# fluent/chunkio

Hardware: AMD Instinct MI355X
Metric: device-resident CRC32 GB/s over N×400KB chunks; % HBM-read roofline (higher is better)
Workload: dtype u8

## Files before the change

chunkio_amd/csrc/cio_diag.h:

```cpp
#ifndef CIO_DIAG_H
#define CIO_DIAG_H



#ifndef CIO_DIAG_HALF_REPLICAS
#define CIO_DIAG_HALF_REPLICAS 0
#endif

#ifndef CIO_ABLATE_LOADS
#define CIO_ABLATE_LOADS 0
#endif

#ifndef CIO_DIAG_NO_ARRIVAL
#define CIO_DIAG_NO_ARRIVAL 0
#endif

#ifndef CIO_DIAG_TAIL
#define CIO_DIAG_TAIL 0
#endif

#ifndef CIO_LDS_FOLD
#define CIO_LDS_FOLD 1
#endif

#ifndef CIO_AHEAD_PEEL
#define CIO_AHEAD_PEEL 1
#endif

#ifndef CIO_SMALL_SLOTS
#define CIO_SMALL_SLOTS 1
#endif
#ifndef CIO_SMALL_EXP
#define CIO_SMALL_EXP 0
#endif

#ifndef CIO_HEAD_ALIGN
#define CIO_HEAD_ALIGN 128
#endif

#ifndef CIO_SMALL_NIBFOLD
#define CIO_SMALL_NIBFOLD 0
#endif


#ifndef CIO_SHA1_GROUP
#define CIO_SHA1_GROUP 4
#endif
#ifndef CIO_SHA1_SCHED_WAVES
#define CIO_SHA1_SCHED_WAVES 1
#endif
#ifndef CIO_SHA1_CHAINS
#define CIO_SHA1_CHAINS 32
#endif
#ifndef CIO_SHA1_READ_AT
#define CIO_SHA1_READ_AT 0
#endif
#ifndef CIO_SHA1_GROUP8
#define CIO_SHA1_GROUP8 8
#endif
// ... 26 lines not shown
```

chunkio_amd/csrc/cio_gpu_internal.h:

```cpp
#ifndef CIOA_GPU_INTERNAL_H
#define CIOA_GPU_INTERNAL_H

#include <hip/hip_runtime.h>
#include <stdint.h>
#include <string>
#include <vector>

#include "cio_diag.h"
#include "crc32_host.h"
#include "chunkio_amd/cio_crc32_gpu.h"

namespace cioa {

constexpr int kWave = 64;
constexpr int kGran = 16;
constexpr int kSub = 4;
constexpr int kRow = kWave * kGran;
constexpr int kStep = kSub * kRow;
constexpr int kThreads = 1024;
constexpr uint32_t kWavesPerWg = kThreads / kWave;
constexpr uint32_t kWfFold = 1u, kWfPublish = 2u;
constexpr int kX8Count = 2 * kStep;
constexpr uint32_t kSliceBytes = 131072;
constexpr uint32_t kShiftBytes = 32768;
// ... 5 lines not shown
    uint64_t a;
    uint64_t vlen;
    uint64_t g;
    uint32_t nsteps;
    uint32_t h;
    uint32_t npieces;
    uint32_t w0, w1;
    uint32_t pad;
};
static_assert(sizeof(ChunkDesc) == 48, "desc layout");

struct WaveStart {
    ChunkDesc d;
    uint32_t c;
    uint32_t pad[3];
};
static_assert(sizeof(WaveStart) == 64, "wave start layout");

struct DeviceState {
    bool ready = false;
    int cus = 0;
    uint32_t *slice = nullptr;
    uint32_t *shift = nullptr;
    uint32_t *x8 = nullptr;
    uint32_t *xinv8 = nullptr;
};

struct PlanHost {
    std::vector<ChunkDesc> desc;
    std::vector<WaveStart> ws;
    std::vector<uint32_t> tiny;
    std::vector<uint32_t> pfac;
    uint64_t S = 0, bytes = 0;
};

constexpr int kMaxDev = 64;

extern thread_local std::string g_err;
int fail(const char *what, hipError_t e = hipSuccess);
int device_state(DeviceState **out);
void plan_init(cio_crc32_plan *p, DeviceState *st, size_t n);
const char *plan_build(PlanHost &ph, const uint64_t *offs, const uint64_t *lens, size_t n, uint32_t W);
int plan_exec_impl(const cio_crc32_plan *p, const void *dev_base, const uint32_t *dev_seeds,
                   uint32_t *dev_out, const uint32_t *cid, hipStream_t s,
                   hipEvent_t ev0 = nullptr, hipEvent_t ev1 = nullptr);


constexpr int kDevHdrS = 0, kDevHdrNtiny = 1, kDevHdrBytes = 2, kDevHdrStatus = 3, kDevHdrWords = 4;
constexpr uint32_t kPlanBlock = 1024;

struct PlanBlockSum {
    uint64_t steps, bytes;
    uint32_t ntiny, err;
};

int devplan_launch_planner(const cio_crc32_devplan *dp, uint64_t dev_bytes, const uint64_t *dev_offs,
                           const uint64_t *dev_lens, size_t n, uint32_t *dev_status, hipStream_t s);
int devplan_crc_launch(const cio_crc32_plan *p, const unsigned long long *hdr, const void *dev_base,
                       const uint32_t *dev_seeds, uint32_t *dev_out, size_t n, hipStream_t s);

}

#define HIP_TRY(expr, what)                             \
    do {                                                   \
        hipError_t e_ = (expr);                            \
        if (e_ != hipSuccess) return cioa::fail(what, e_); \
    } while (0)

struct cio_crc32_plan {
    uint32_t n = 0;
    uint64_t S = 0;
    uint32_t W = 0;
    uint32_t grid = 0;
    uint32_t ntiny = 0;
    int prio = 1;
    uint64_t ustride = 0, ua0 = 0, uvlen = 0;
    uint32_t unsteps = 0, uh = 0;
    bool small = false;
    bool ahead = false;
    bool l64 = false;
    bool l64_small = false;
    unsigned long long *stamps = nullptr;
    uint64_t bytes = 0;
    cioa::ChunkDesc *desc = nullptr;
    cioa::WaveStart *wstart = nullptr;
    uint32_t *tiny = nullptr;
    unsigned long long *partials = nullptr;
    uint32_t *counters = nullptr;
    uint32_t *pfac = nullptr;
    cioa::DeviceState *st = nullptr;
};

struct cio_crc32_devplan {
    cio_crc32_plan *p = nullptr;
    uint32_t max_chunks = 0;
    cioa::PlanBlockSum *bsum = nullptr;
    unsigned long long *hdr = nullptr;
    uint64_t *roffs = nullptr, *rlens = nullptr;
    uint32_t *rcrc = nullptr;
};

#endif
```

chunkio_amd/csrc/crc32_gpu.hip:

```cpp

#include <hip/hip_runtime.h>
#include <stdint.h>
#include <string.h>
#include <stdio.h>
#include <stdlib.h>
#include <memory>
#include <mutex>
#include <shared_mutex>
#include <vector>
#include <string>
#include <algorithm>

#include <type_traits>

#include "cio_gpu_internal.h"

using namespace cioa;

namespace {


constexpr uint32_t cx_multmodp(uint32_t a, uint32_t b)
{
    uint32_t p = 0;
// ... 23 lines not shown
{
    uint32_t p = 0;
#pragma unroll
    for (int i = 31; i >= 0; --i) {
        p ^= b & (0u - ((a >> i) & 1u));
        b = (b >> 1) ^ (CIOA_POLY & (0u - (b & 1u)));
    }
    return p;
}

template <uint32_t C>
struct MulCols {
    uint32_t v[32];
    constexpr MulCols() : v{}
    {
        for (int j = 0; j < 32; ++j) {
            v[j] = cx_multmodp(C, 1u << j);
        }
    }
};

template <uint32_t C>
__device__ __forceinline__ uint32_t mulconst(uint32_t b)
{
    constexpr MulCols<C> K;
    uint32_t p[4] = {0u, 0u, 0u, 0u};
#pragma unroll
    for (int j = 0; j < 32; ++j) {
        p[j & 3] = __builtin_amdgcn_bitop3_b32(p[j & 3], 0u - ((b >> j) & 1u), K.v[j], 0x78);
    }
    return __builtin_amdgcn_bitop3_b32(p[0], p[1], p[2], 0x96) ^ p[3];
}

template <bool TREE>
__device__ __forceinline__ uint32_t fold_full(const uint32_t (&s)[kSub])
{
    constexpr uint32_t kXRow = cx_xpow8n(kRow);
    uint32_t h = s[0];
#pragma unroll
    for (int q = 1; q < kSub; ++q) {
        h = (TREE ? mulconst<kXRow>(h) : multmodp(kXRow, h)) ^ s[q];
    }
    return h;
}

__device__ __forceinline__ uint64_t div_u52(uint64_t x, uint64_t d)
{
    uint64_t q = (uint64_t) ((double) x / (double) d);
    if (q * d > x) {
        q -= 1;
    } else if ((q + 1) * d <= x) {
        q += 1;
    }
    return q;
}

__device__ __forceinline__ uint64_t uniform_u64(uint64_t v)
{
    const uint32_t lo = __builtin_amdgcn_readfirstlane((uint32_t) v);
    const uint32_t hi = __builtin_amdgcn_readfirstlane((uint32_t) (v >> 32));
    return ((uint64_t) hi << 32) | lo;
}

__device__ __forceinline__ uint64_t split_point(uint64_t w, uint64_t X, uint64_t W)
{
    if ((W & (W - 1)) == 0) {
// ... 113 lines not shown
}

constexpr int kE = 1024 / kThreads;
static_assert(kE == 1, "one slice and one shift entry per thread");

template <bool STAMPS = false, bool SHIFT = true>
__device__ __forceinline__ void write_tables(char *lds, uint32_t tid, const uint32_t (&tab_v)[kE],
                                             const uint32_t (&tab_sv)[kE], unsigned long long *ts = nullptr)
{
    const uint32_t k = tid >> 8, b = tid & 255u, lane = tid & 63u;
    const uint32_t srow = (k >> 1) * 65536u + b * 256u + (k & 1u) * 128u;
    const uint4 sv = make_uint4(tab_v[0], tab_v[0], tab_v[0], tab_v[0]);
#pragma unroll
    for (int i = 0; i < 8; ++i) {
        *reinterpret_cast<uint4 *>(lds + srow + 16u * ((lane + (uint32_t) i) & 7u)) = sv;
    }
    if (SHIFT) {
        const uint32_t hrow = kShiftOff + k * 8192u + b * 32u;
        const uint4 hv = make_uint4(tab_sv[0], tab_sv[0], tab_sv[0], tab_sv[0]);
#pragma unroll
        for (int i = 0; i < 2; ++i) {
            *reinterpret_cast<uint4 *>(lds + hrow + 16u * ((lane + (uint32_t) i) & 1u)) = hv;
        }
    }
    if (STAMPS) {
        ts[0] = __builtin_amdgcn_s_memrealtime();
        ts[1] = ts[0];
    }
}

struct StepRegs {
    uint4 q[kSub];
};

__device__ __forceinline__ void load_step(StepRegs &r, const uint8_t *cbase, uint64_t jj,
                                          uint64_t vlen, uint32_t lane)
{
    const uint64_t b0 = jj * kStep + (uint64_t) lane * kGran;
    const uint64_t last = (vlen - 1) & ~15ull;
#pragma unroll
    for (int q = 0; q < kSub; ++q) {
#if CIO_ABLATE_LOADS
        const uint64_t a = min(b0 + (uint64_t) q * kRow, last) + (uint64_t) (uintptr_t) cbase;
        r.q[q] = make_uint4((uint32_t) a, (uint32_t) (a >> 7) * 0x9E3779B9u, (uint32_t) a ^ 0x5bd1e995u,
                            (uint32_t) (a >> 3) + 0x7f4a7c15u);
#else
        r.q[q] = ldg16(cbase + min(b0 + (uint64_t) q * kRow, last));
#endif
    }
}

__device__ __forceinline__ void load_step64(StepRegs &r, const uint8_t *cbase, uint64_t jj, uint32_t lane)
{
    const uint64_t b0 = jj * kStep + (uint64_t) (64u * (lane & 15u) + 16u * (lane >> 4));
#pragma unroll
    for (int q = 0; q < kSub; ++q) {
        r.q[q] = ldg16(cbase + b0 + (uint64_t) q * kRow);
    }
}

__device__ __forceinline__ void load_step64c(StepRegs &r, const uint8_t *cbase, uint64_t jj, uint64_t vlen,
                                             uint32_t lane)
{
    const uint64_t b0 = jj * kStep + (uint64_t) (64u * (lane & 15u) + 16u * (lane >> 4));
    const uint64_t last = (vlen - 1) & ~15ull;
#pragma unroll
// ... 179 lines not shown
    }
}

__device__ __forceinline__ void tiny_chunks(const char *lds, uint32_t lb_lo, const uint8_t *base,
                                            const ChunkDesc *desc, const uint32_t *tiny,
                                            const uint32_t *seeds, uint32_t *out, const uint32_t *cid,
                                            uint32_t ntiny, uint32_t wave, uint32_t lane, uint32_t W)
{
    for (uint64_t t = (uint64_t) wave * kWave + lane; t < ntiny; t += (uint64_t) W * kWave) {
        const uint32_t c = tiny[t];
        const ChunkDesc d = desc[c];
        const uint32_t oc = cid ? cid[c] : c;
        uint32_t st = seeds ? seeds[oc] : 0xffffffffu;
        const uint8_t *p = base + d.a + d.h;
        const uint32_t len = (uint32_t) (d.vlen - d.h);
        for (uint32_t i = 0; i < len; ++i) {
            st = byte_step(lds, lb_lo, st, p[i]);
        }
        out[oc] = st;
    }
}

__device__ __forceinline__ void rotate_prio(uint32_t slot_group, uint64_t it)
{
    switch ((slot_group + (uint32_t) it) & 3u) {
    case 0: __builtin_amdgcn_s_setprio(0); break;
    case 1: __builtin_amdgcn_s_setprio(1); break;
    case 2: __builtin_amdgcn_s_setprio(2); break;
    default: __builtin_amdgcn_s_setprio(3); break;
    }
}

template <bool STAMPS = false, int PRIO = 1, bool UNIFORM = false, bool AHEAD = false, bool L64 = false,
          bool DEVHDR = false>
__global__ void __launch_bounds__(kThreads, 1)
crc32_stream_kernel(const uint8_t *base, uint64_t S_arg, uint64_t ustride, uint64_t ua0, uint64_t uvlen,
                    uint32_t W, uint32_t unsteps, uint32_t uh, uint32_t n,
                    const ChunkDesc *__restrict__ desc,
                    const WaveStart *__restrict__ wstart, const uint32_t *__restrict__ tiny,
                    const uint32_t *__restrict__ seeds, uint32_t *out, const uint32_t *__restrict__ cid,
                    unsigned long long *__restrict__ partials, uint32_t *__restrict__ counters,
                    const uint32_t *__restrict__ g_slice, const uint32_t *__restrict__ g_shift,
                    const uint32_t *__restrict__ g_x8, const uint32_t *__restrict__ pfac,
                    uint32_t ntiny_arg, unsigned long long *stamps)
{
    static_assert(!DEVHDR || (!STAMPS && !UNIFORM && !AHEAD), "device-planned batches take the general path");
    __shared__ __attribute__((aligned(16))) char lds[kLdsBytes];
    const uint32_t tid = threadIdx.x;
    const uint64_t S = DEVHDR ? uniform_u64(stamps[kDevHdrS]) : S_arg;
    const uint32_t ntiny = DEVHDR ? __builtin_amdgcn_readfirstlane((uint32_t) stamps[kDevHdrNtiny]) : ntiny_arg;
    unsigned long long t_entry = 0, t_tables = 0, t_stream = 0, t_first = 0, t_mid = 0, t_issued = 0;
    unsigned long long t_wt[2] = {0, 0}, t_step1 = 0, t_arrived = 0, t_bar1 = 0, t_bar2 = 0, t_folded = 0;
    if (STAMPS) {
        t_entry = __builtin_amdgcn_s_memrealtime();
    }

    const uint32_t wave = __builtin_amdgcn_readfirstlane(blockIdx.x * (kThreads / kWave) + (tid >> 6));
    const uint32_t lane = tid & 63u;
    const uint32_t lb_lo = (lane & kSliceRepMask) << 2;
    const uint32_t lb_hi = lb_lo | 0x10000u;
    const uint32_t lrep = (lane & kShiftRepMask) << 2;
    const uint32_t slot_group = __builtin_amdgcn_readfirstlane((tid >> 6) >> 2);
    const uint64_t g0 = uniform_u64(wave_start(wave, S, W));
    const uint64_t gend = uniform_u64(wave_start((uint64_t) wave + 1, S, W));
    const bool active = g0 < gend;

    uint32_t c = 0, lc = 0, c0 = 0;
    ChunkDesc d = {}, ld = {};
    uint32_t j = 0, lj = 0;
    uint64_t nload = 0;
    if (active) {
        if (UNIFORM) {
            c = __builtin_amdgcn_readfirstlane((uint32_t) split_point(wave, n, W));
            d.a = ua0 + (uint64_t) c * ustride;
            d.vlen = uvlen;
            d.g = (uint64_t) c * unsteps;
            d.nsteps = unsteps;
            d.h = uh;
        } else {
// ... 37 lines not shown
        if (nload > 0) {
            --nload;
            if (++lj == ld.nsteps && nload > 0) {
                if (UNIFORM) {
                    ++lc;
                    ld.a += ustride;
                    ld.g += unsteps;
                } else {
                    do {
                        ++lc;
                        ld = desc[lc];
                    } while (ld.nsteps == 0);
                }
                lj = 0;
            }
        }
    };

    auto build_tables = [&]() {
        uint32_t tab_v[kE], tab_sv[kE];
#pragma unroll
        for (int e = 0; e < kE; ++e) {
            const uint32_t idx = tid + (uint32_t) kThreads * e;
            table_entries<L64 ? cx_xpow8n(kStep - 64) : kXStepShift>(__builtin_amdgcn_readfirstlane(idx >> 8),
                                                                     idx & 255u, tab_v[e], tab_sv[e]);
        }
        write_tables<STAMPS>(lds, tid, tab_v, tab_sv, t_wt);
    };
    StepRegs cur, nxt;
    issue(cur);
    __builtin_amdgcn_sched_barrier(0);
    uint64_t ar_g = 0;
    uint32_t ar_ns = 0, ar_np = 0, ar_w0 = 0, ar_w1 = 0;
    if (CIO_DIAG_NO_ARRIVAL < 2) {
        const ChunkDesc &ad = desc[min(c0 + lane, n - 1)];
        ar_g = ad.g;
        ar_ns = ad.nsteps;
        ar_np = ad.npieces;
        ar_w0 = ad.w0;
        ar_w1 = ad.w1;
    }
    const uint32_t xl = g_x8[L64 ? 64u * (63u - lane) : kRow - (lane + 1) * kGran];
    const uint32_t *wwords = pfac + (W + n + 1);
    const uint32_t wfl = CIO_LDS_FOLD ? load_lane_u32(wwords + wave) : 0u;
    const uint32_t wlast = load_lane_u32(wwords + W + wave);
    uint32_t fold_own = 0, pub = 0;
    __builtin_amdgcn_sched_barrier(0);
    if (STAMPS) {
        t_issued = __builtin_amdgcn_s_memrealtime();
    }

    build_tables();
    __syncthreads();
    if (STAMPS) {
        t_tables = __builtin_amdgcn_s_memrealtime();
    }

    if (active) {
        uint32_t s[kSub] = {0u, 0u, 0u, 0u};
        uint64_t e[kSub] = {0ull, 0ull, 0ull, 0ull};
        uint32_t xlast = 0;
        uint32_t full_end = (uint32_t) (d.vlen / kStep);
        uint32_t seed = (j == 0) ? (seeds ? seeds[cid ? cid[c] : c] : 0xffffffffu) : 0u;
        uint64_t g = g0;

        auto crc_step = [&](StepRegs &r) -> bool {
            {
                if (L64 && (AHEAD || j < full_end)) {
                    const uint32_t h0 = step_shift(lds, lrep, s[0]);
                    transpose64(r);
                    if (j == 0) {
                        if (AHEAD) {
                            r.q[0].x ^= lane == 0 ? seed : 0u;
                        } else {
                            r.q[0] = head_fix(r.q[0], 4u * lane, d.h, seed);
                            r.q[1] = head_fix(r.q[1], 4u * lane + 1u, d.h, seed);
                            if (CIO_HEAD_ALIGN > 16) {
                                r.q[2] = head_fix(r.q[2], 4u * lane + 2u, d.h, seed);
                                r.q[3] = head_fix(r.q[3], 4u * lane + 3u, d.h, seed);
                            }
                        }
                    }
                    uint32_t st = block16(lds, lb_lo, lb_hi, h0, r.q[0]);
#pragma unroll
                    for (int q = 1; q < kSub; ++q) {
                        st = block16(lds, lb_lo, lb_hi, st, r.q[q]);
                    }
                    s[0] = st;
                    if (!AHEAD) {
                        e[0] = (uint64_t) j * kStep + 64ull * (lane + 1);
                    }
                } else if (L64) {
                    transpose64(r);
                    slow_compute64(lds, lb_lo, lb_hi, lrep, r, j, d.vlen, d.h, seed, lane, s[0], e[0]);
                } else if (AHEAD || j < full_end) {
                    uint32_t h[kSub];
#pragma unroll
                    for (int q = 0; q < kSub; ++q) {
                        h[q] = step_shift(lds, lrep, s[q]);
                    }
                    if (j == 0) {
                        r.q[0] = head_fix(r.q[0], lane, d.h, seed);
                    }
#pragma unroll
                    for (int q = 0; q < kSub; ++q) {
                        s[q] = block16(lds, lb_lo, lb_hi, h[q], r.q[q]);
                    }
                    if (!AHEAD) {
                        const uint64_t e0 = (uint64_t) j * kStep + (uint64_t) (lane + 1) * kGran;
#pragma unroll
                        for (int q = 0; q < kSub; ++q) {
                            e[q] = e0 + (uint64_t) q * kRow;
                        }
                    }
                } else {
                    slow_compute(lds, lb_lo, lb_hi, lrep, r, j, d.vlen, d.h, seed, lane, s, e);
                }
                ++g;
                ++j;
                return j == d.nsteps || g == gend;
            }
        };
        auto piece_end = [&]() {
            {
                {
                    uint32_t contrib;
                    if (AHEAD || j <= full_end) {
                        uint32_t a = j < d.nsteps ? xlast : xl;
                        asm volatile("" : "+v"(a));
                        contrib = multmodp(a, L64 ? s[0] : fold_full<UNIFORM>(s));
                    } else {
                        const uint64_t pend = min((uint64_t) j * kStep, d.vlen);
                        contrib = 0;
#pragma unroll
                        for (int q = 0; q < kSub; ++q) {
                            const uint64_t dist = e[q] < pend ? pend - e[q] : 0;
                            contrib ^= s[q] ? multmodp(g_x8[min(dist, (uint64_t) (kX8Count - 1))], s[q]) : 0u;
                        }
                    }
                    contrib = wave_xor(contrib);
                    if (d.g >= g0 && j == d.nsteps) {
                        if (lane == 0) {
                            out[cid ? cid[c] : c] = contrib;
                        }
                    } else if (j == d.nsteps && (wfl & kWfFold)) {
                        fold_own = contrib;
                    } else if (j < d.nsteps && (wfl & kWfPublish)) {
                        pub = contrib;
                    } else {
                        __hip_atomic_store(&partials[(uint64_t) wave + c], (unsigned long long) contrib,
                                           __ATOMIC_RELAXED, __HIP_MEMORY_SCOPE_AGENT);
                    }
                    if (g < gend) {
                        if (UNIFORM) {
                            ++c;
                            d.a += ustride;
                            d.g += unsteps;
                        } else {
                            do {
                                ++c;
                                d = desc[c];
                            } while (d.nsteps == 0);
                        }
                        j = 0;
#pragma unroll
                        for (int q = 0; q < kSub; ++q) {
                            s[q] = 0u;
                            e[q] = 0ull;
                        }
                        full_end = (uint32_t) (d.vlen / kStep);
                        seed = seeds ? seeds[cid ? cid[c] : c] : 0xffffffffu;
                    }
                }
            }
        };

        if (STAMPS) {
            t_first = __builtin_amdgcn_s_memrealtime();
        }
        const uint64_t iters = gend - g0;
        const uint64_t it_f = iters > 1 ? 1 : 0;
        if (AHEAD) {
            auto landed = [](StepRegs &r) {
                asm volatile("" : "+v"(r.q[0].x), "+v"(r.q[0].y), "+v"(r.q[0].z), "+v"(r.q[0].w),
                                  "+v"(r.q[1].x), "+v"(r.q[1].y), "+v"(r.q[1].z), "+v"(r.q[1].w),
                                  "+v"(r.q[2].x), "+v"(r.q[2].y), "+v"(r.q[2].z), "+v"(r.q[2].w),
                                  "+v"(r.q[3].x), "+v"(r.q[3].y), "+v"(r.q[3].z), "+v"(r.q[3].w));
            };
            auto half = [&](uint64_t it, StepRegs &use, StepRegs &fill, auto refill) {
                if (PRIO) {
                    rotate_prio(slot_group, it);
                }
                if (it == it_f) {
                    uint32_t wl = wlast;
                    asm volatile("" : "+v"(wl));
                    xlast = multmodp(wl, xl);
                }
                landed(use);
                if (decltype(refill)::value) {
                    issue(fill);
                }
                if (crc_step(use)) {
                    piece_end();
                }
                if (STAMPS && it == 0) {
                    t_step1 = __builtin_amdgcn_s_memrealtime();
                }
                if (STAMPS && it == iters / 2) {
                    t_mid = __builtin_amdgcn_s_memrealtime();
                }
            };
            using Refill = std::true_type;
#if CIO_AHEAD_PEEL
            using NoRefill = std::false_type;
            uint64_t it = 0;
            for (; it + 2 < iters; it += 2) {
                half(it, cur, nxt, Refill());
                half(it + 1, nxt, cur, Refill());
            }
            if (iters - it == 2) {
                half(it, cur, nxt, Refill());
                half(it + 1, nxt, cur, NoRefill());
            } else if (iters - it == 1) {
                half(it, cur, nxt, NoRefill());
            }
#else
            for (uint64_t it = 0; it < iters; it += 2) {
                half(it, cur, nxt, Refill());
                if (it + 1 < iters) {
                    half(it + 1, nxt, cur, Refill());
                }
            }
#endif
        }
        for (uint64_t it = 0; !AHEAD && it < iters; ++it) {
            if (PRIO) {
                rotate_prio(slot_group, it);
            }
            if (it == it_f) {
                uint32_t wl = wlast;
                asm volatile("" : "+v"(wl));
                xlast = multmodp(wl, xl);
            }
            const bool pe = crc_step(cur);
            if (STAMPS && it == 0) {
                t_step1 = __builtin_amdgcn_s_memrealtime();
            }
            if (nload > 0) {
                issue(cur);
            }
            if (pe) {
                piece_end();
            }
            if (STAMPS && it == iters / 2) {
                t_mid = __builtin_amdgcn_s_memrealtime();
            }
        }
        if (PRIO) {
            __builtin_amdgcn_s_setprio(0);
        }

        asm volatile("s_waitcnt vmcnt(0)" ::: "memory");
        if (STAMPS) {
            t_stream = __builtin_amdgcn_s_memrealtime();
        }
        for (uint32_t ac = c0; !CIO_DIAG_NO_ARRIVAL;) {
            const uint32_t idx = ac + lane;
            const bool inb = idx < n;
            const bool whole = ar_g >= g0 && ar_g + ar_ns <= gend;
            const bool local = CIO_LDS_FOLD && (ar_w0 ^ ar_w1) < kWavesPerWg;
            const bool member = inb && ar_ns != 0 && ar_g < gend && !whole && !local;
            const bool stop = !inb || (ar_ns != 0 && ar_g >= gend);
            uint32_t old = 0;
            if (member) {
                old = __hip_atomic_fetch_add(&counters[idx], 1u, __ATOMIC_RELAXED, __HIP_MEMORY_SCOPE_AGENT);
            }
            for (uint64_t fin = __ballot(member && old + 1 == ar_np); fin; fin &= fin - 1) {
                const uint32_t b = (uint32_t) __builtin_ctzll(fin);
                const uint32_t fc = ac + b;
                fold_chunk(__builtin_amdgcn_readlane(ar_w0, b), __builtin_amdgcn_readlane(ar_w1, b), fc,
                           cid ? cid[fc] : fc, lane, partials, pfac, out, counters);
            }
            if (__ballot(stop)) {
                break;
            }
            ac += kWave;
            const ChunkDesc &ad = desc[min(ac + lane, n - 1)];
            ar_g = ad.g;
            ar_ns = ad.nsteps;
            ar_np = ad.npieces;
            ar_w0 = ad.w0;
            ar_w1 = ad.w1;
        }
    }

    if (STAMPS) {
        t_arrived = __builtin_amdgcn_s_memrealtime();
    }
    tiny_chunks(lds, lb_lo, base, desc, tiny, seeds, out, cid, ntiny, wave, lane, W);
    if (CIO_LDS_FOLD) {
        __syncthreads();
        if (STAMPS) {
            t_bar1 = __builtin_amdgcn_s_memrealtime();
        }
        uint32_t *slot = reinterpret_cast<uint32_t *>(lds);
        if (lane == 0) {
            slot[tid >> 6] = pub;
        }
        __syncthreads();
        if (STAMPS) {
            t_bar2 = __builtin_amdgcn_s_memrealtime();
        }
        if (wfl & kWfFold) {
            const uint32_t nb = (wfl >> 8) & 0xffu;
            uint32_t a = 0;
            if (lane < kWavesPerWg && lane >= kWavesPerWg - nb) {
                a = slot[(tid >> 6) + lane - kWavesPerWg];
            }
            a = wave_xor(a) ^ fold_own;
            if (lane == 0) {
                out[cid ? cid[c0] : c0] = a;
            }
        }
        if (STAMPS) {
            t_folded = __builtin_amdgcn_s_memrealtime();
        }
    }
#if CIO_DIAG_TAIL == 1
    {
        const unsigned long long t0 = __builtin_amdgcn_s_memrealtime();
        while (__builtin_amdgcn_s_memrealtime() - t0 < 500) {
            __builtin_amdgcn_s_sleep(10);
        }
    }
#elif CIO_DIAG_TAIL == 2
    __syncthreads();
#endif
    if (STAMPS && lane == 0) {
        uint32_t hw_id, xcc_id;
        asm volatile("s_getreg_b32 %0, hwreg(HW_REG_HW_ID)" : "=s"(hw_id));
        asm volatile("s_getreg_b32 %0, hwreg(HW_REG_XCC_ID)" : "=s"(xcc_id));
        stamps[kStampWords * wave + 0] = t_entry;
        stamps[kStampWords * wave + 1] = t_tables;
        stamps[kStampWords * wave + 2] = t_stream;
        stamps[kStampWords * wave + 3] = __builtin_amdgcn_s_memrealtime();
        stamps[kStampWords * wave + 4] = hw_id;
        stamps[kStampWords * wave + 5] = xcc_id;
        stamps[kStampWords * wave + 6] = t_first;
        stamps[kStampWords * wave + 7] = t_mid;
        stamps[kStampWords * wave + 8] = t_issued;
        stamps[kStampWords * wave + 9] = t_wt[0];
        stamps[kStampWords * wave + 10] = t_wt[1];
        stamps[kStampWords * wave + 11] = t_step1;
        stamps[kStampWords * wave + 12] = t_arrived;
// ... 569 lines not shown
        std::vector<uint32_t> xinv8(kStep);
        uint32_t xm8 = 0x80000000u;
        for (int i = 0; i < 8; ++i) {
            xm8 = cioa_multmodp(xm8, (CIOA_POLY << 1) | 1u);
        }
        xinv8[0] = 0x80000000u;
        for (int d = 1; d < kStep; ++d) {
            xinv8[d] = cioa_multmodp(xinv8[d - 1], xm8);
        }
        HIP_TRY(hipMalloc(&st.xinv8, kStep * sizeof(uint32_t)), "hipMalloc(xinv8)");
        HIP_TRY(hipMemcpy(st.xinv8, xinv8.data(), kStep * sizeof(uint32_t), hipMemcpyHostToDevice),
                "upload xinv8");
        st.ready = true;
    }
    *out = &st;
    return CIO_OK;
}

}

extern "C" {

const char *cio_gpu_last_error(void)
{
    return g_err.c_str();
}

const char *cio_gpu_version(void)
{
#define CIO_STR2(x) #x
#define CIO_STR(x) CIO_STR2(x)
    return "chunkio_amd crc32 v9 gfx950 stream(l64-lanes permlane-transpose issue-ahead<=64steps pre-shift prio-rotate "
           "coalesced-nt division-free-start slice4-lds32x perm direct-whole preshifted-partials wg-lds-fold "
           "head-align=" CIO_STR(CIO_HEAD_ALIGN) ") "
           "small(4x16B dpp-reduce bitop3-fold prio-rotate) "
           "host(nt-staging graduated-groups pread-bounce multi-device vpclmul-crc_update small-batch-route) "
           "sha1(2-schedule-waves 4-block-handover continuation)";
}

int cio_gpu_init(void)
{
    DeviceState *st;
    return device_state(&st);
}

void cio_crc32_plan_destroy(cio_crc32_plan *p)
{
    if (!p) {
        return;
    }
    (void) hipFree(p->desc);
    (void) hipFree(p->wstart);
    (void) hipFree(p->tiny);
    (void) hipFree(p->partials);
    (void) hipFree(p->counters);
    (void) hipFree(p->pfac);
    (void) hipFree(p->stamps);
    delete p;
}

}

namespace cioa {

void plan_init(cio_crc32_plan *p, DeviceState *st, size_t n)
{
// ... 73 lines not shown
    const size_t nslots = (size_t) W + n + 1;
    ph.pfac.assign(nslots + 2 * (size_t) W, 0u);
    if (S > 0) {
        size_t c = 0;
        for (uint32_t w = 0; w < W; w++) {
            const uint64_t g0 = ((uint64_t) w * S) / W;
            const uint64_t g1 = ((uint64_t) (w + 1) * S) / W;
            while (c < n && (ph.desc[c].nsteps == 0 || ph.desc[c].g + ph.desc[c].nsteps <= g0)) {
                c++;
            }
            wc[w] = (uint32_t) std::min(c, n - 1);
            if (g0 == g1) {
                continue;
            }
            for (size_t k = c; k < n && ph.desc[k].g < g1; k++) {
                ChunkDesc &d = ph.desc[k];
                if (d.nsteps) {
                    if (d.npieces == 0) {
                        d.w0 = w;
                    }
                    d.w1 = w;
                    wl[w] = (uint32_t) k;
                    d.npieces++;
                    const uint64_t pend = std::min(std::min(g1 - d.g, (uint64_t) d.nsteps) * (uint64_t) kStep,
                                                   d.vlen);
                    ph.pfac[w + k] = factor(d.vlen - pend);
                }
            }
        }
    }
    auto local = [](const ChunkDesc &d) {
        return d.npieces > 1 && d.w0 / kWavesPerWg == d.w1 / kWavesPerWg;
    };
    for (uint32_t w = 0; S > 0 && w < W; w++) {
        const uint64_t g0 = ((uint64_t) w * S) / W;
        const uint64_t g1 = ((uint64_t) (w + 1) * S) / W;
        if (g0 == g1) {
            continue;
        }
        uint32_t f = 0;
        const ChunkDesc &first = ph.desc[wc[w]];
        if (first.g < g0 && first.g + first.nsteps <= g1 && local(first)) {
            f |= kWfFold | ((w - first.w0) << 8);
        }
        const ChunkDesc &last = ph.desc[wl[w]];
        const bool nonfinal = last.g + last.nsteps > g1;
        if (nonfinal && local(last)) {
            f |= kWfPublish;
        }
        ph.pfac[nslots + w] = f;
        ph.pfac[nslots + W + w] = nonfinal ? ph.pfac[w + wl[w]] : 0x80000000u;
    }
    ph.ws.assign(W, WaveStart{});
    for (uint32_t w = 0; w < W; w++) {
        ph.ws[w].c = wc[w];
        if (n) {
            ph.ws[w].d = ph.desc[wc[w]];
        }
    }
    return nullptr;
}

}

namespace {

// ... 59 lines not shown
            oversub = true;
            ph = std::move(ph4);
        }
    }
    {
        const char *r = cioa_diag_getenv("CIO_GPU_ANTICAMP");
        const bool on = !(r && atoi(r) == 0);
        const char *mx = cioa_diag_getenv("CIO_GPU_ANTICAMP_MAX");
        const bool small_batch = ph.S > 0 && ph.S == (uint64_t) n - ph.tiny.size();
        const uint64_t wmax = mx ? strtoull(mx, nullptr, 10) : small_batch ? 128 : 64;
        const uint64_t w = p->W ? ph.S / p->W : 0;
        const bool any_grid = r && atoi(r) == 2;
        if (on && (!oversub || any_grid) && !cioa_diag_getenv("CIO_GPU_GRID") && p->grid % 32 == 0 && ph.S % p->W == 0 &&
            w % 16 == 0 &&
            w > 0 && w <= wmax) {
            const uint32_t g2 = p->grid / 32 * 31;
            PlanHost ph2;
            if (plan_build(ph2, offs, lens, n, g2 * (kThreads / kWave)) == nullptr) {
                p->grid = g2;
                p->W = g2 * (kThreads / kWave);
                ph = std::move(ph2);
            }
        }
    }
    p->S = ph.S;
    p->bytes = ph.bytes;
    p->ntiny = (uint32_t) ph.tiny.size();
    p->ahead = p->unsteps != 0 && p->uh == 0 && p->uvlen % kStep == 0;
    bool short_ranges = p->S <= 64ull * p->W;
    if (const char *r = cioa_diag_getenv("CIO_GPU_AHEAD")) {
        short_ranges = atoi(r) != 0;
    }
    p->ahead = p->ahead && short_ranges;

    p->small = ph.S > 0 && ph.S == (uint64_t) n - ph.tiny.size();
    if (const char *r = cioa_diag_getenv("CIO_GPU_SMALL")) {
        p->small = p->small && atoi(r) != 0;
    }
    if (const char *r = cioa_diag_getenv("CIO_GPU_STAMPS")) {
        if (atoi(r) > 0 && hipMalloc(&p->stamps, (size_t) p->W * kStampWords * sizeof(unsigned long long)) != hipSuccess) {
            p->stamps = nullptr;
        }
    }
    hipError_t e;
    const size_t npart = ph.pfac.size();
    if ((e = hipMalloc(&p->desc, ph.desc.size() * sizeof(ChunkDesc))) != hipSuccess ||
        (e = hipMalloc(&p->wstart, ph.ws.size() * sizeof(WaveStart))) != hipSuccess ||
        (e = hipMalloc(&p->tiny, std::max<size_t>(1, ph.tiny.size()) * sizeof(uint32_t))) != hipSuccess ||
        (e = hipMalloc(&p->partials, npart * sizeof(unsigned long long))) != hipSuccess ||
        (e = hipMalloc(&p->counters, std::max<size_t>(1, n) * sizeof(uint32_t))) != hipSuccess ||
        (e = hipMalloc(&p->pfac, npart * sizeof(uint32_t))) != hipSuccess ||
        (e = hipMemcpy(p->desc, ph.desc.data(), ph.desc.size() * sizeof(ChunkDesc), hipMemcpyHostToDevice)) != hipSuccess ||
        (e = hipMemcpy(p->wstart, ph.ws.data(), ph.ws.size() * sizeof(WaveStart), hipMemcpyHostToDevice)) != hipSuccess ||
        (ph.tiny.size() && (e = hipMemcpy(p->tiny, ph.tiny.data(), ph.tiny.size() * sizeof(uint32_t), hipMemcpyHostToDevice)) != hipSuccess) ||
        (e = hipMemset(p->partials, 0, npart * sizeof(unsigned long long))) != hipSuccess ||
        (e = hipMemset(p->counters, 0, std::max<size_t>(1, n) * sizeof(uint32_t))) != hipSuccess ||
        (e = hipMemcpy(p->pfac, ph.pfac.data(), npart * sizeof(uint32_t), hipMemcpyHostToDevice)) != hipSuccess) {
        cio_crc32_plan_destroy(p);
        return fail("cio_crc32_plan_create: device allocation/upload", e);
    }
    *out = p;
    return CIO_OK;
}

struct cio_crc32_ring {
    std::vector<cio_crc32_plan *> plans;
// ... 151 lines not shown

uint32_t cio_crc32_plan_workgroups(const cio_crc32_plan *p)
{
    return p ? p->grid : 0;
}

const char *cio_crc32_plan_kernel(const cio_crc32_plan *p)
{
    return (p && p->small) ? "crc32_small_kernel" : "crc32_stream_kernel";
}


int cio_crc32_plan_exec_events(const cio_crc32_plan *p, const void *dev_base,
                               const uint32_t *dev_seeds, uint32_t *dev_out, void *stream,
                               void *ev_piece_start, void *ev_piece_stop)
{
    return plan_exec_impl(p, dev_base, dev_seeds, dev_out, nullptr,
                          reinterpret_cast<hipStream_t>(stream),
                          reinterpret_cast<hipEvent_t>(ev_piece_start),
                          reinterpret_cast<hipEvent_t>(ev_piece_stop));
}

int cio_crc32_plan_exec(const cio_crc32_plan *p, const void *dev_base, const uint32_t *dev_seeds,
                        uint32_t *dev_out, void *stream)
{
    return plan_exec_impl(p, dev_base, dev_seeds, dev_out, nullptr,
                          reinterpret_cast<hipStream_t>(stream));
}

}

using StreamKernel = decltype(&crc32_stream_kernel<false, 1, false>);

static StreamKernel select_kernel(int prio, bool stamps, bool uniform, bool ahead, bool l64)
{
    if (ahead) {
        if (l64) {
            if (stamps) {
                return crc32_stream_kernel<true, 1, true, true, true>;
            }
            return prio ? crc32_stream_kernel<false, 1, true, true, true>
                        : crc32_stream_kernel<false, 0, true, true, true>;
        }
        return prio ? crc32_stream_kernel<false, 1, true, true> : crc32_stream_kernel<false, 0, true, true>;
    }
    if (l64 && !stamps) {
        return prio ? crc32_stream_kernel<false, 1, false, false, true>
                    : crc32_stream_kernel<false, 0, false, false, true>;
    }
    switch ((prio ? 4 : 0) + (stamps ? 2 : 0) + (uniform ? 1 : 0)) {
    case 0: return crc32_stream_kernel<false, 0, false>;
    case 1: return crc32_stream_kernel<false, 0, true>;
    case 2: return crc32_stream_kernel<true, 0, false>;
    case 3: return crc32_stream_kernel<true, 0, true>;
    case 4: return crc32_stream_kernel<false, 1, false>;
    case 5: return crc32_stream_kernel<false, 1, true>;
    case 6: return crc32_stream_kernel<true, 1, false>;
    default: return crc32_stream_kernel<true, 1, true>;
    }
}


int cioa::plan_exec_impl(const cio_crc32_plan *p, const void *dev_base, const uint32_t *dev_seeds,
                         uint32_t *dev_out, const uint32_t *cid, hipStream_t s,
                         hipEvent_t ev0, hipEvent_t ev1)
{
    if (!p) {
        return fail("cio_crc32_plan_exec: null plan");
    }
    if (p->n == 0) {
        return CIO_OK;
    }
    if (!dev_base || !dev_out) {
        return fail("cio_crc32_plan_exec: null buffer");
    }
    const DeviceState *st = p->st;
    if (ev0) {
        HIP_TRY(hipEventRecord(ev0, s), "hipEventRecord");
    }
    if (p->small && !cid) {
        auto sk = p->l64_small ? (p->unsteps ? (dev_seeds ? crc32_small_kernel<true, true, true>
                                                    : crc32_small_kernel<true, false, true>)
                                       : (dev_seeds ? crc32_small_kernel<false, true, true>
                                                    : crc32_small_kernel<false, false, true>))
                         : (p->unsteps ? (dev_seeds ? crc32_small_kernel<true, true> : crc32_small_kernel<true, false>)
                                       : (dev_seeds ? crc32_small_kernel<false, true>
                                                    : crc32_small_kernel<false, false>));
        hipLaunchKernelGGL(sk, dim3(p->grid), dim3(kThreads), 0, s,
                           reinterpret_cast<const uint8_t *>(dev_base), p->ustride, p->ua0, p->uvlen, p->uh,
                           p->W, p->n, p->ntiny, st->x8, p->desc, p->tiny, dev_seeds, dev_out, st->xinv8);
        HIP_TRY(hipGetLastError(), "crc32_small_kernel launch");
        if (ev1) {
            HIP_TRY(hipEventRecord(ev1, s), "hipEventRecord");
        }
        return CIO_OK;
    }
    auto kern = select_kernel(p->prio, p->stamps != nullptr, p->unsteps != 0, p->ahead && (!p->stamps || p->l64),
                              p->l64);
    hipLaunchKernelGGL(kern, dim3(p->grid), dim3(kThreads), 0, s,
                       reinterpret_cast<const uint8_t *>(dev_base), p->S, p->ustride, p->ua0, p->uvlen,
                       p->W, p->unsteps, p->uh, p->n, p->desc, p->wstart, p->tiny,
                       dev_seeds, dev_out, cid, p->partials, p->counters, st->slice, st->shift,
                       st->x8, p->pfac, p->ntiny, p->stamps);
    HIP_TRY(hipGetLastError(), "crc32_stream_kernel launch");
    if (ev1) {
        HIP_TRY(hipEventRecord(ev1, s), "hipEventRecord");
    }
    return CIO_OK;
}

int cioa::devplan_crc_launch(const cio_crc32_plan *p, const unsigned long long *hdr, const void *dev_base,
                             const uint32_t *dev_seeds, uint32_t *dev_out, size_t n, hipStream_t s)
{
    const DeviceState *st = p->st;
    StreamKernel kern = p->l64 ? (p->prio ? crc32_stream_kernel<false, 1, false, false, true, true>
                                          : crc32_stream_kernel<false, 0, false, false, true, true>)
                               : (p->prio ? crc32_stream_kernel<false, 1, false, false, false, true>
                                          : crc32_stream_kernel<false, 0, false, false, false, true>);
    hipLaunchKernelGGL(kern, dim3(p->grid), dim3(kThreads), 0, s,
                       reinterpret_cast<const uint8_t *>(dev_base), (uint64_t) 0, (uint64_t) 0, (uint64_t) 0,
                       (uint64_t) 0, p->W, 0u, 0u, (uint32_t) n, p->desc, p->wstart, p->tiny,
                       dev_seeds, dev_out, (const uint32_t *) nullptr, p->partials, p->counters, st->slice,
                       st->shift, st->x8, p->pfac, 0u, const_cast<unsigned long long *>(hdr));
    HIP_TRY(hipGetLastError(), "crc32_stream_kernel (device-planned) launch");
    return CIO_OK;
}

extern "C" {

int cio_crc32_batch_dev(const void *dev_base, const uint64_t *offs, const uint64_t *lens,
                        const uint32_t *dev_seeds, uint32_t *dev_out, size_t n, void *stream)
// ... 217 lines not shown
```

Before: 6196.

## Add edge-free kernel instantiation for workgroup-local plans with premultiplied last-step columns

Adds an EDGE template variant of the stream kernel, chosen on the host when every chunk either fits in one piece or stays within a single workgroup, no tiny chunks exist and no cid remap is used. That variant skips the cross-workgroup arrival loop, the final vmcnt(0) wait, the tiny-chunk pass and the global partial publishes. It also builds the multiply-by-x^n column table for the last step ahead of time so the closing multmodp leaves the critical tail. The cost is more template instantiations, extra VGPRs for the 32-entry column table, and correctness that depends on the host-side eligibility check.

```diff
diff --git a/chunkio_amd/csrc/cio_diag.h b/chunkio_amd/csrc/cio_diag.h
--- a/chunkio_amd/csrc/cio_diag.h
+++ b/chunkio_amd/csrc/cio_diag.h
@@ -25,6 +25,16 @@
 
 #ifndef CIO_AHEAD_PEEL
 #define CIO_AHEAD_PEEL 1
+#endif
+
+#ifndef CIO_EDGE_FREE
+#define CIO_EDGE_FREE 1
+#endif
+#ifndef CIO_EDGE_PREMUL
+#define CIO_EDGE_PREMUL 1
+#endif
+#ifndef CIO_EDGE_EARLY2
+#define CIO_EDGE_EARLY2 0
 #endif
 
 #ifndef CIO_SMALL_SLOTS
diff --git a/chunkio_amd/csrc/cio_gpu_internal.h b/chunkio_amd/csrc/cio_gpu_internal.h
--- a/chunkio_amd/csrc/cio_gpu_internal.h
+++ b/chunkio_amd/csrc/cio_gpu_internal.h
@@ -61,6 +61,7 @@
     std::vector<uint32_t> tiny;
     std::vector<uint32_t> pfac;
     uint64_t S = 0, bytes = 0;
+    bool wg_local = false;
 };
 
 constexpr int kMaxDev = 64;
@@ -107,6 +108,7 @@
     uint32_t unsteps = 0, uh = 0;
     bool small = false;
     bool ahead = false;
+    bool edge_free = false;
     bool l64 = false;
     bool l64_small = false;
     unsigned long long *stamps = nullptr;
diff --git a/chunkio_amd/csrc/crc32_gpu.hip b/chunkio_amd/csrc/crc32_gpu.hip
--- a/chunkio_amd/csrc/crc32_gpu.hip
+++ b/chunkio_amd/csrc/crc32_gpu.hip
@@ -79,6 +79,25 @@
     return __builtin_amdgcn_bitop3_b32(p[0], p[1], p[2], 0x96) ^ p[3];
 }
 
+__device__ __forceinline__ void mul_cols(uint32_t a, uint32_t (&m)[32])
+{
+    m[31] = a;
+#pragma unroll
+    for (int j = 31; j > 0; --j) {
+        m[j - 1] = (m[j] >> 1) ^ (CIOA_POLY & (0u - (m[j] & 1u)));
+    }
+}
+
+__device__ __forceinline__ uint32_t mul_by_cols(const uint32_t (&m)[32], uint32_t b)
+{
+    uint32_t p[4] = {0u, 0u, 0u, 0u};
+#pragma unroll
+    for (int j = 0; j < 32; ++j) {
+        p[j & 3] = __builtin_amdgcn_bitop3_b32(p[j & 3], 0u - ((b >> j) & 1u), m[j], 0x78);
+    }
+    return __builtin_amdgcn_bitop3_b32(p[0], p[1], p[2], 0x96) ^ p[3];
+}
+
 template <bool TREE>
 __device__ __forceinline__ uint32_t fold_full(const uint32_t (&s)[kSub])
 {
@@ -258,6 +277,14 @@
 struct StepRegs {
     uint4 q[kSub];
 };
+
+__device__ __forceinline__ void step_landed(StepRegs &r)
+{
+    asm volatile("" : "+v"(r.q[0].x), "+v"(r.q[0].y), "+v"(r.q[0].z), "+v"(r.q[0].w),
+                      "+v"(r.q[1].x), "+v"(r.q[1].y), "+v"(r.q[1].z), "+v"(r.q[1].w),
+                      "+v"(r.q[2].x), "+v"(r.q[2].y), "+v"(r.q[2].z), "+v"(r.q[2].w),
+                      "+v"(r.q[3].x), "+v"(r.q[3].y), "+v"(r.q[3].z), "+v"(r.q[3].w));
+}
 
 __device__ __forceinline__ void load_step(StepRegs &r, const uint8_t *cbase, uint64_t jj,
                                           uint64_t vlen, uint32_t lane)
@@ -503,7 +530,7 @@
 }
 
 template <bool STAMPS = false, int PRIO = 1, bool UNIFORM = false, bool AHEAD = false, bool L64 = false,
-          bool DEVHDR = false>
+          bool DEVHDR = false, bool EDGE = false>
 __global__ void __launch_bounds__(kThreads, 1)
 crc32_stream_kernel(const uint8_t *base, uint64_t S_arg, uint64_t ustride, uint64_t ua0, uint64_t uvlen,
                     uint32_t W, uint32_t unsteps, uint32_t uh, uint32_t n,
@@ -516,6 +543,10 @@
                     uint32_t ntiny_arg, unsigned long long *stamps)
 {
     static_assert(!DEVHDR || (!STAMPS && !UNIFORM && !AHEAD), "device-planned batches take the general path");
+    static_assert(!EDGE || (UNIFORM && AHEAD), "the edge-free promise is made for issue-ahead plans only");
+    constexpr bool kNoEdges = EDGE && CIO_EDGE_FREE;
+    constexpr bool kPremul = EDGE && CIO_EDGE_PREMUL && CIO_AHEAD_PEEL;
+    constexpr bool kEarly2 = EDGE && CIO_EDGE_EARLY2;
     __shared__ __attribute__((aligned(16))) char lds[kLdsBytes];
     const uint32_t tid = threadIdx.x;
     const uint64_t S = DEVHDR ? uniform_u64(stamps[kDevHdrS]) : S_arg;
@@ -619,7 +650,7 @@
     __builtin_amdgcn_sched_barrier(0);
     uint64_t ar_g = 0;
     uint32_t ar_ns = 0, ar_np = 0, ar_w0 = 0, ar_w1 = 0;
-    if (CIO_DIAG_NO_ARRIVAL < 2) {
+    if (CIO_DIAG_NO_ARRIVAL < 2 && !kNoEdges) {
         const ChunkDesc &ad = desc[min(c0 + lane, n - 1)];
         ar_g = ad.g;
         ar_ns = ad.nsteps;
@@ -638,6 +669,10 @@
     }
 
     build_tables();
+    if (kEarly2) {
+        step_landed(cur);
+        issue(nxt);
+    }
     __syncthreads();
     if (STAMPS) {
         t_tables = __builtin_amdgcn_s_memrealtime();
@@ -648,8 +683,9 @@
         uint64_t e[kSub] = {0ull, 0ull, 0ull, 0ull};
         uint32_t xlast = 0;
         uint32_t full_end = (uint32_t) (d.vlen / kStep);
-        uint32_t seed = (j == 0) ? (seeds ? seeds[cid ? cid[c] : c] : 0xffffffffu) : 0u;
+        uint32_t seed = (j == 0) ? (seeds ? seeds[!kNoEdges && cid ? cid[c] : c] : 0xffffffffu) : 0u;
         uint64_t g = g0;
+        uint32_t mcol[32];
 
         auto crc_step = [&](StepRegs &r) -> bool {
             {
@@ -708,11 +744,13 @@
                 return j == d.nsteps || g == gend;
             }
         };
-        auto piece_end = [&]() {
+        auto piece_end = [&](auto last_step) {
             {
                 {
                     uint32_t contrib;
-                    if (AHEAD || j <= full_end) {
+                    if (kPremul && decltype(last_step)::value) {
+                        contrib = mul_by_cols(mcol, L64 ? s[0] : fold_full<UNIFORM>(s));
+                    } else if (AHEAD || j <= full_end) {
                         uint32_t a = j < d.nsteps ? xlast : xl;
                         asm volatile("" : "+v"(a));
                         contrib = multmodp(a, L64 ? s[0] : fold_full<UNIFORM>(s));
@@ -728,11 +766,11 @@
                     contrib = wave_xor(contrib);
                     if (d.g >= g0 && j == d.nsteps) {
                         if (lane == 0) {
-                            out[cid ? cid[c] : c] = contrib;
+                            out[!kNoEdges && cid ? cid[c] : c] = contrib;
                         }
                     } else if (j == d.nsteps && (wfl & kWfFold)) {
                         fold_own = contrib;
-                    } else if (j < d.nsteps && (wfl & kWfPublish)) {
+                    } else if (kNoEdges || (j < d.nsteps && (wfl & kWfPublish))) {
                         pub = contrib;
                     } else {
                         __hip_atomic_store(&partials[(uint64_t) wave + c], (unsigned long long) contrib,
@@ -756,7 +794,7 @@
                             e[q] = 0ull;
                         }
                         full_end = (uint32_t) (d.vlen / kStep);
-                        seed = seeds ? seeds[cid ? cid[c] : c] : 0xffffffffu;
+                        seed = seeds ? seeds[!kNoEdges && cid ? cid[c] : c] : 0xffffffffu;
                     }
                 }
             }
@@ -774,7 +812,7 @@
                                   "+v"(r.q[2].x), "+v"(r.q[2].y), "+v"(r.q[2].z), "+v"(r.q[2].w),
                                   "+v"(r.q[3].x), "+v"(r.q[3].y), "+v"(r.q[3].z), "+v"(r.q[3].w));
             };
-            auto half = [&](uint64_t it, StepRegs &use, StepRegs &fill, auto refill) {
+            auto half = [&](uint64_t it, StepRegs &use, StepRegs &fill, auto refill, auto last, auto pre) {
                 if (PRIO) {
                     rotate_prio(slot_group, it);
                 }
@@ -783,12 +821,23 @@
                     asm volatile("" : "+v"(wl));
                     xlast = multmodp(wl, xl);
                 }
-                landed(use);
+                if (kPremul && decltype(last)::value) {
+                    uint32_t a = j + 1 < d.nsteps ? xlast : xl;
+                    asm volatile("" : "+v"(a));
+                    mul_cols(a, mcol);
+                    __builtin_amdgcn_sched_barrier(0);
+                }
+                if (!decltype(pre)::value) {
+                    landed(use);
+                }
+                if (STAMPS && it + 1 == iters) {
+                    t_wt[1] = __builtin_amdgcn_s_memrealtime();
+                }
                 if (decltype(refill)::value) {
                     issue(fill);
                 }
                 if (crc_step(use)) {
-                    piece_end();
+                    piece_end(last);
                 }
                 if (STAMPS && it == 0) {
                     t_step1 = __builtin_amdgcn_s_memrealtime();
@@ -798,24 +847,40 @@
                 }
             };
             using Refill = std::true_type;
+            using No = std::false_type;
 #if CIO_AHEAD_PEEL
             using NoRefill = std::false_type;
+            using Last = std::true_type;
             uint64_t it = 0;
+            if (kEarly2) {
+                half(0, cur, nxt, NoRefill(), No(), std::true_type());
+                for (it = 1; it + 2 < iters; it += 2) {
+                    half(it, nxt, cur, Refill(), No(), No());
+                    half(it + 1, cur, nxt, Refill(), No(), No());
+                }
+                if (iters - it == 2) {
+                    half(it, nxt, cur, Refill(), No(), No());
+                    half(it + 1, cur, nxt, NoRefill(), Last(), No());
+                } else if (iters - it == 1) {
+                    half(it, nxt, cur, NoRefill(), Last(), No());
+                }
+            } else {
             for (; it + 2 < iters; it += 2) {
-                half(it, cur, nxt, Refill());
-                half(it + 1, nxt, cur, Refill());
+                half(it, cur, nxt, Refill(), No(), No());
+                half(it + 1, nxt, cur, Refill(), No(), No());
             }
             if (iters - it == 2) {
-                half(it, cur, nxt, Refill());
-                half(it + 1, nxt, cur, NoRefill());
+                half(it, cur, nxt, Refill(), No(), No());
+                half(it + 1, nxt, cur, NoRefill(), Last(), No());
             } else if (iters - it == 1) {
-                half(it, cur, nxt, NoRefill());
+                half(it, cur, nxt, NoRefill(), Last(), No());
+            }
             }
 #else
             for (uint64_t it = 0; it < iters; it += 2) {
-                half(it, cur, nxt, Refill());
+                half(it, cur, nxt, Refill(), No(), No());
                 if (it + 1 < iters) {
-                    half(it + 1, nxt, cur, Refill());
+                    half(it + 1, nxt, cur, Refill(), No(), No());
                 }
             }
 #endif
@@ -837,7 +902,7 @@
                 issue(cur);
             }
             if (pe) {
-                piece_end();
+                piece_end(std::false_type());
             }
             if (STAMPS && it == iters / 2) {
                 t_mid = __builtin_amdgcn_s_memrealtime();
@@ -847,11 +912,13 @@
             __builtin_amdgcn_s_setprio(0);
         }
 
-        asm volatile("s_waitcnt vmcnt(0)" ::: "memory");
+        if (!kNoEdges) {
+            asm volatile("s_waitcnt vmcnt(0)" ::: "memory");
+        }
         if (STAMPS) {
             t_stream = __builtin_amdgcn_s_memrealtime();
         }
-        for (uint32_t ac = c0; !CIO_DIAG_NO_ARRIVAL;) {
+        for (uint32_t ac = c0; !CIO_DIAG_NO_ARRIVAL && !kNoEdges;) {
             const uint32_t idx = ac + lane;
             const bool inb = idx < n;
             const bool whole = ar_g >= g0 && ar_g + ar_ns <= gend;
@@ -884,7 +951,9 @@
     if (STAMPS) {
         t_arrived = __builtin_amdgcn_s_memrealtime();
     }
-    tiny_chunks(lds, lb_lo, base, desc, tiny, seeds, out, cid, ntiny, wave, lane, W);
+    if (!kNoEdges) {
+        tiny_chunks(lds, lb_lo, base, desc, tiny, seeds, out, cid, ntiny, wave, lane, W);
+    }
     if (CIO_LDS_FOLD) {
         __syncthreads();
         if (STAMPS) {
@@ -906,7 +975,7 @@
             }
             a = wave_xor(a) ^ fold_own;
             if (lane == 0) {
-                out[cid ? cid[c0] : c0] = a;
+                out[!kNoEdges && cid ? cid[c0] : c0] = a;
             }
         }
         if (STAMPS) {
@@ -1542,6 +1611,7 @@
 #define CIO_STR(x) CIO_STR2(x)
     return "chunkio_amd crc32 v9 gfx950 stream(l64-lanes permlane-transpose issue-ahead<=64steps pre-shift prio-rotate "
            "coalesced-nt division-free-start slice4-lds32x perm direct-whole preshifted-partials wg-lds-fold "
+           "edge-free-instantiation "
            "head-align=" CIO_STR(CIO_HEAD_ALIGN) ") "
            "small(4x16B dpp-reduce bitop3-fold prio-rotate) "
            "host(nt-staging graduated-groups pread-bounce multi-device vpclmul-crc_update small-batch-route) "
@@ -1681,6 +1751,11 @@
     auto local = [](const ChunkDesc &d) {
         return d.npieces > 1 && d.w0 / kWavesPerWg == d.w1 / kWavesPerWg;
     };
+    ph.wg_local = S > 0 && ph.tiny.empty();
+    for (size_t i = 0; i < n && ph.wg_local; i++) {
+        const ChunkDesc &d = ph.desc[i];
+        ph.wg_local = d.npieces == 1 || local(d);
+    }
     for (uint32_t w = 0; S > 0 && w < W; w++) {
         const uint64_t g0 = ((uint64_t) w * S) / W;
         const uint64_t g1 = ((uint64_t) (w + 1) * S) / W;
@@ -1806,6 +1881,10 @@
         short_ranges = atoi(r) != 0;
     }
     p->ahead = p->ahead && short_ranges;
+    p->edge_free = p->ahead && ph.wg_local && p->ntiny == 0;
+    if (const char *r = cioa_diag_getenv("CIO_GPU_EDGE")) {
+        p->edge_free = p->edge_free && atoi(r) != 0;
+    }
 
     p->small = ph.S > 0 && ph.S == (uint64_t) n - ph.tiny.size();
     if (const char *r = cioa_diag_getenv("CIO_GPU_SMALL")) {
@@ -2023,8 +2102,44 @@
 
 using StreamKernel = decltype(&crc32_stream_kernel<false, 1, false>);
 
-static StreamKernel select_kernel(int prio, bool stamps, bool uniform, bool ahead, bool l64)
-{
+static thread_local bool g_last_edge = false;
+
+extern "C" {
+
+int cioa_debug_plan_edge_free(const cio_crc32_plan *p)
+{
+    return p && p->edge_free;
+}
+
+int cioa_debug_last_launch_edge_free(void)
+{
+    return g_last_edge;
+}
+
+int cioa_debug_plan_wg_local(const uint64_t *offs, const uint64_t *lens, size_t n, uint32_t W)
+{
+    PlanHost ph;
+    if (plan_build(ph, offs, lens, n, W) != nullptr) {
+        return -1;
+    }
+    return ph.wg_local;
+}
+
+}
+
+static StreamKernel select_kernel(int prio, bool stamps, bool uniform, bool ahead, bool l64, bool edge)
+{
+    if (ahead && edge) {
+        if (l64) {
+            if (stamps) {
+                return crc32_stream_kernel<true, 1, true, true, true, false, true>;
+            }
+            return prio ? crc32_stream_kernel<false, 1, true, true, true, false, true>
+                        : crc32_stream_kernel<false, 0, true, true, true, false, true>;
+        }
+        return prio ? crc32_stream_kernel<false, 1, true, true, false, false, true>
+                    : crc32_stream_kernel<false, 0, true, true, false, false, true>;
+    }
     if (ahead) {
         if (l64) {
             if (stamps) {
@@ -2066,6 +2181,7 @@
         return fail("cio_crc32_plan_exec: null buffer");
     }
     const DeviceState *st = p->st;
+    g_last_edge = false;
     if (ev0) {
         HIP_TRY(hipEventRecord(ev0, s), "hipEventRecord");
     }
@@ -2086,8 +2202,10 @@
         }
         return CIO_OK;
     }
-    auto kern = select_kernel(p->prio, p->stamps != nullptr, p->unsteps != 0, p->ahead && (!p->stamps || p->l64),
-                              p->l64);
+    const bool ahead = p->ahead && (!p->stamps || p->l64);
+    const bool edge = ahead && p->edge_free && !cid;
+    g_last_edge = edge;
+    auto kern = select_kernel(p->prio, p->stamps != nullptr, p->unsteps != 0, ahead, p->l64, edge);
     hipLaunchKernelGGL(kern, dim3(p->grid), dim3(kThreads), 0, s,
                        reinterpret_cast<const uint8_t *>(dev_base), p->S, p->ustride, p->ua0, p->uvlen,
                        p->W, p->unsteps, p->uh, p->n, p->desc, p->wstart, p->tiny,
```

Result: no change. 6257 (median of 6 runs) (+1.0%).
